# yaoyx689/RigGS

Measured on AMD Instinct MI355X. Metric: train iters/sec (deform+raster fwd+bwd), 300k Gaussians @800x800, higher is better.
Workload: dtype f32; 1 GPU; 300k Gaussians / 24-joint skeleton / 800x800, LBS-only, SH degree 3, anisotropic, one frame per GPU per step; num_gaussians=300000, num_joints=24, tile_instances_R=1963607, tile_lists=canonical: upstream's ceil(3 sigma) squares (the library default), parallelism=frames x1, launch=hipGraph replay

## Files before the change

riggs_amd/csrc/binning.hip:

```cpp
#include <stdlib.h>
#include <type_traits>
#include "raster_internal.h"
#include "color_job.h"

namespace riggs {


__device__ __forceinline__ int rect_tile(const ushort4 rc, int l, int grid_x) {
  const int w = rc.z - rc.x;
  const int ry = (int)(((float)l + 0.5f) * __builtin_amdgcn_rcpf((float)w));
  const int rx = l - ry * w;
  return (rc.y + ry) * grid_x + rc.x + rx;
}

__device__ __forceinline__ ushort4 unpack_rect(const uint2 w) {
  return make_ushort4((unsigned short)(w.x & 0xFFFFu), (unsigned short)(w.x >> 16), (unsigned short)(w.y & 0xFFFFu), (unsigned short)(w.y >> 16));
}
__device__ __forceinline__ ushort4 load_rect(const ushort4* p) { return unpack_rect(*reinterpret_cast<const uint2*>(p)); }

__global__ __launch_bounds__(1024) void bin_count_kernel(int N, int T, int grid_x, int g_per_block,
                                                        const uint32_t* __restrict__ order,
                                                        const ushort4* __restrict__ rect,
                                                        ushort4* __restrict__ srect ,
                                                        uint32_t* __restrict__ table) {
  extern __shared__ uint32_t s_hist[];
  for (int t = threadIdx.x; t < T; t += blockDim.x) s_hist[t] = 0u;
  __syncthreads();
  const int first = blockIdx.x * g_per_block;
  const int end = min(N, first + g_per_block);
  for (int s = first + threadIdx.x; s < end; s += blockDim.x) {
    const uint32_t g = order[s];
    const ushort4 rc = load_rect(rect + g);
    srect[s] = rc;
    if (rc.z == rc.x) continue;
    for (int y = rc.y; y < rc.w; y++)
      for (int x = rc.x; x < rc.z; x++) atomicAdd(&s_hist[y * grid_x + x], 1u);
  }
  __syncthreads();
  uint32_t* row = table + (size_t)blockIdx.x * T;
  for (int t = threadIdx.x; t < T; t += blockDim.x) row[t] = s_hist[t];
}

#define SCAN_SEG 16
#define SCAN_KEEP 32
__device__ __forceinline__ void bin_scan_body(int T, int n_chunks, uint32_t* __restrict__ table,
                                              uint32_t* __restrict__ tile_count) {
  __shared__ uint32_t s_seg[SCAN_SEG][64];
  const int tl = threadIdx.x & 63, seg = threadIdx.x >> 6;
  const int t = blockIdx.x * 64 + tl;
  const int per = (n_chunks + SCAN_SEG - 1) / SCAN_SEG;
  const int b0 = seg * per, b1 = min(n_chunks, b0 + per);
  uint32_t sum = 0;
  if (per <= SCAN_KEEP) {
    uint32_t v[SCAN_KEEP];
#pragma unroll
    for (int i = 0; i < SCAN_KEEP; i++) v[i] = (t < T && b0 + i < b1) ? table[(size_t)(b0 + i) * T + t] : 0u;
#pragma unroll
    for (int i = 0; i < SCAN_KEEP; i++) sum += v[i];
    s_seg[seg][tl] = sum;
    __syncthreads();
    uint32_t run = 0;
    for (int s2 = 0; s2 < seg; s2++) run += s_seg[s2][tl];
    if (t < T) {
#pragma unroll
      for (int i = 0; i < SCAN_KEEP; i++) {
        if (b0 + i < b1) table[(size_t)(b0 + i) * T + t] = run;
        run += v[i];
      }
      if (seg == SCAN_SEG - 1) tile_count[t] = run;
    }
    return;
  }
  if (t < T) for (int b = b0; b < b1; b++) sum += table[(size_t)b * T + t];
  s_seg[seg][tl] = sum;
  __syncthreads();
  uint32_t run = 0;
  for (int s2 = 0; s2 < seg; s2++) run += s_seg[s2][tl];
  if (t < T) {
    for (int b = b0; b < b1; b++) { const uint32_t c = table[(size_t)b * T + t]; table[(size_t)b * T + t] = run; run += c; }
    if (seg == SCAN_SEG - 1) tile_count[t] = run;
  }
}
__global__ __launch_bounds__(1024) void bin_scan_kernel(int T, int n_chunks, uint32_t* __restrict__ table,
                                                        uint32_t* __restrict__ tile_count) {
  bin_scan_body(T, n_chunks, table, tile_count);
}

__device__ void bin_offsets_body(int T, int64_t cap, const uint32_t* __restrict__ tile_count, const BinOut o,
                                 const uint32_t* __restrict__ total_src = nullptr, int n_total_src = 0) {
  uint2* __restrict__ ranges = o.ranges;
  uint32_t* __restrict__ slot_base = o.slot_base;
  uint32_t* __restrict__ tile_max = o.tile_max;
  uint32_t* __restrict__ counters = o.counters;
  uint32_t* __restrict__ fwd_items = o.fwd_items;
  uint32_t* __restrict__ fwd_empty = o.fwd_empty;
  uint32_t* __restrict__ fwd_ctr = o.fwd_ctr;
  __shared__ uint32_t s_wave[16], s_wwave[16];
  __shared__ uint32_t s_carry, s_wcarry;
  __shared__ uint32_t s_hist[33], s_cur[33], s_nempty;
  const int nthr = (int)blockDim.x;
  const int tid = threadIdx.x, lane = tid & 63, wave = tid >> 6;
  __shared__ int s_slot;
  if (tid == 0) { s_carry = 0u; s_nempty = 0u; s_wcarry = 0u; s_slot = RIGGS_HIST_SLOTS; }
  if (tid < 33) s_hist[tid] = 0u;
  const uint32_t slot_words = riggs_hist_slot_words((uint32_t)T);
  uint32_t* const hist_hdr = o.walk_hist;
  __syncthreads();
  if (o.viewmatrix) {
    for (int sl = tid; sl < RIGGS_HIST_SLOTS; sl += nthr) {
      const uint32_t* hs = hist_hdr + RIGGS_HIST_HDR + (size_t)sl * slot_words;
      bool ok = hs[T] == o.hist_stamp;
      for (int e = 0; e < 16 && ok; e++) ok = fabsf(o.viewmatrix[e] - __uint_as_float(hs[T + 2 + e])) <= o.view_tol;
      if (ok) atomicMin(&s_slot, sl);
    }
  } else if (tid == 0 && hist_hdr[RIGGS_HIST_HDR + T] == o.hist_stamp) s_slot = 0;
  __syncthreads();
  const bool slot_found = s_slot < RIGGS_HIST_SLOTS;
  const uint32_t cursor = hist_hdr[0];
  const int slot = slot_found ? s_slot : (o.viewmatrix ? (int)(cursor % RIGGS_HIST_SLOTS) : 0);
  uint32_t* __restrict__ walk_hist = hist_hdr + RIGGS_HIST_HDR + (size_t)slot * slot_words;
  const bool have_hist = o.wide_tiles > 0u && slot_found;
  __syncthreads();
  if (tid == 0) {
    hist_hdr[1] = (uint32_t)slot;
    if (!slot_found && o.viewmatrix) hist_hdr[0] = cursor + 1u;
  }
  uint32_t my_len[8];
#pragma unroll
  for (int k = 0; k < 8; k++) my_len[k] = 0u;
  for (int base = 0, pass = 0; base < T; base += nthr, pass++) {
    const int t = base + tid;
    const uint32_t c = (t < T) ? tile_count[t] : 0u;
    uint32_t v = c;
    for (int o2 = 1; o2 < 64; o2 <<= 1) {
      const uint32_t u = (uint32_t)__shfl_up((int)v, o2);
      if (lane >= o2) v += u;
    }
    const uint32_t prev = (have_hist && t < T) ? walk_hist[t] : 0u;
// ... 30 lines not shown
    __shared__ uint32_t s_tot;
    if (tid == 0) s_tot = 0u;
    __syncthreads();
    uint32_t part = 0;
    for (int k = tid; k < n_total_src; k += nthr) part += total_src[k];
    for (int o2 = 32; o2 > 0; o2 >>= 1) part += (uint32_t)__shfl_xor((int)part, o2);
    if (lane == 0) atomicAdd(&s_tot, part);
    __syncthreads();
    if (tid == 0) s_carry = s_tot;
    __syncthreads();
  }
  if (tid == 0) {
    const uint32_t R = s_carry;
    ranges[T] = make_uint2(0u, 0u);
    tile_max[T] = 0u;
    slot_base[T] = ((uint32_t)min((int64_t)R, cap) >> 6) + (uint32_t)T;
    counters[0] = R;
    counters[1] = (counters[1] & 2u) | (((int64_t)R > cap) ? 1u : 0u);
  }
  __syncthreads();
  if (tid < 32) {
    const uint32_t n_wide = s_hist[32];
    const uint32_t h = s_hist[31 - tid];
    uint32_t v = h;
    for (int o2 = 1; o2 < 32; o2 <<= 1) {
      const uint32_t u = (uint32_t)__shfl_up((int)v, o2);
      if (tid >= o2) v += u;
    }
    s_cur[31 - tid] = n_wide + v - h;
    if (tid == 0) s_cur[32] = 0u;
    if (tid == 31) { fwd_ctr[0] = n_wide + v; fwd_ctr[1] = n_wide; fwd_ctr[2] = s_nempty; fwd_ctr[64] = 0u; }
  }
  __syncthreads();
  auto emit = [&](uint32_t t, uint32_t len) { fwd_items[atomicAdd(&s_cur[(walk_hist[t] >> 31) ? 32 : 31 - __builtin_clz(len)], 1u)] = t; };
#pragma unroll
  for (int k = 0; k < 8; k++) {
    const int t = k * nthr + tid;
    if (t < T && my_len[k] > 0u) emit((uint32_t)t, my_len[k]);
  }
  for (int t = 8 * nthr + tid; t < T; t += nthr) {
    const uint2 r = ranges[t];
    if (r.y > r.x) emit((uint32_t)t, r.y - r.x);
  }
}

__global__ __launch_bounds__(1024) void bin_scatter_kernel(int N, int T, int grid_x, int64_t cap, int g_per_block, int g_per_wave,
                                                          const uint32_t* __restrict__ order,
                                                          const ushort4* __restrict__ srect ,
                                                          const uint32_t* __restrict__ table,
                                                          const uint32_t* __restrict__ tile_count,
                                                          uint32_t* __restrict__ point_list,
                                                          uint32_t* __restrict__ tile_keys, const BinOut out,
                                                          const int n_main, const ColorJob* __restrict__ job_rec, const int job_gpb) {
  extern __shared__ uint32_t s_mem[];
  if ((int)blockIdx.x == n_main) {
    bin_offsets_body(T, cap, tile_count, out);
    return;
  }
  if ((int)blockIdx.x > n_main) {
    const ColorJob job = *job_rec;
    color_block(job, (int)blockIdx.x - n_main - 1, job_gpb, reinterpret_cast<float*>(s_mem));
    return;
  }
  const int W = blockDim.x >> 6;
  uint32_t* s_base = s_mem;
  const int Tpad = (T + 1) & ~1;
  unsigned short* s_rel = reinterpret_cast<unsigned short*>(s_mem + T);
  uint32_t* s_rel32 = s_mem + T;
  const int tid = threadIdx.x, lane = tid & 63, wave = tid >> 6;
  const int first = blockIdx.x * g_per_block + wave * g_per_wave;
  const int end = min(N, min(first + g_per_wave, (blockIdx.x + 1) * g_per_block));
  auto load_batch = [&](int s0, uint32_t& g, uint32_t& n, ushort4& rc) {
    const int s = s0 + lane;
    g = 0u; n = 0u; rc = make_ushort4(0, 0, 0, 0);
    if (s < end) {
      g = order[s];
      rc = srect[s];
      n = (uint32_t)((int)(rc.z - rc.x) * (int)(rc.w - rc.y));
    }
  };
  uint32_t nx_g = 0u;
  uint2 nx_w = make_uint2(0u, 0u);
  if (first + lane < end) { nx_g = order[first + lane]; nx_w = *reinterpret_cast<const uint2*>(srect + first + lane); }
  const uint32_t* row = table + (size_t)blockIdx.x * T;
  uint32_t cq0[4], rq0[4];
#pragma unroll
  for (int k = 0; k < 4; k++) {
    const int t = k * (int)blockDim.x + tid;
    cq0[k] = (t < T) ? tile_count[t] : 0u;
    rq0[k] = (t < T) ? row[t] : 0u;
  }
  for (int e = tid; e < W * (Tpad >> 1); e += blockDim.x) s_rel32[e] = 0u;
  __syncthreads();
  ushort4 nx_rc = unpack_rect(nx_w);
  uint32_t nx_n = (uint32_t)((int)(nx_rc.z - nx_rc.x) * (int)(nx_rc.w - nx_rc.y));
  for (int s0 = first; s0 < end; s0 += 64) {
    uint32_t g = nx_g, n = nx_n;
    ushort4 rc = nx_rc;
    if (s0 != first) load_batch(s0, g, n, rc);
    if (n) {
      uint32_t* hist = s_rel32 + (size_t)wave * (Tpad >> 1);
      for (int y = rc.y; y < rc.w; y++)
        for (int x = rc.x; x < rc.z; x++) {
          const int t = y * grid_x + x;
          atomicAdd(&hist[t >> 1], 1u << (16 * (t & 1)));
        }
    }
  }
  __syncthreads();
  {
    __shared__ uint32_t s_wsum[16];
    __shared__ uint32_t s_run;
    if (tid == 0) s_run = 0u;
    __syncthreads();
    for (int base0 = 0; base0 < T; base0 += 4 * blockDim.x) {
      uint32_t cq[4], rq[4];
#pragma unroll
      for (int k = 0; k < 4; k++) {
        const int t = base0 + k * (int)blockDim.x + tid;
        if (base0 == 0) { cq[k] = cq0[k]; rq[k] = rq0[k]; continue; }
        cq[k] = (t < T) ? tile_count[t] : 0u;
        rq[k] = (t < T) ? row[t] : 0u;
      }
#pragma unroll
      for (int k = 0; k < 4; k++) {
        const int base = base0 + k * (int)blockDim.x;
        if (base >= T) break;
        const int t = base + tid;
        const uint32_t c = cq[k];
        uint32_t v = c;
        for (int o = 1; o < 64; o <<= 1) {
          const uint32_t u = (uint32_t)__shfl_up((int)v, o);
          if (lane >= o) v += u;
        }
        if (lane == 63) s_wsum[wave] = v;
        __syncthreads();
        uint32_t off = s_run;
        for (int w = 0; w < wave; w++) off += s_wsum[w];
        if (t < T) s_base[t] = off + v - c + rq[k];
        __syncthreads();
        if (tid == (int)blockDim.x - 1) s_run = off + v;
        __syncthreads();
      }
    }
  }
  for (int t = tid; t < T; t += blockDim.x) {
    uint32_t run = 0;
    for (int w = 0; w < W; w++) {
      const unsigned short c = s_rel[(size_t)w * Tpad + t];
      s_rel[(size_t)w * Tpad + t] = (unsigned short)run;
      run += c;
    }
  }
  __syncthreads();
  unsigned short* cur = s_rel + (size_t)wave * Tpad;
  const int slot4 = lane >> 4, l16 = lane & 15;
  for (int s0 = first; s0 < end; s0 += 64) {
    const uint32_t cur_g = nx_g, cur_n = nx_n;
    const ushort4 cur_rc = nx_rc;
    if (s0 + 64 < end) load_batch(s0 + 64, nx_g, nx_n, nx_rc);
    const uint64_t live = __builtin_amdgcn_ballot_w64(cur_n != 0u);
    const uint64_t large = __builtin_amdgcn_ballot_w64(cur_n > 16u);
    const uint64_t huge = __builtin_amdgcn_ballot_w64(cur_n > 32u);
    const int pk_xy = (int)cur_rc.x | ((int)cur_rc.y << 16), pk_zw = (int)cur_rc.z | ((int)cur_rc.w << 16);
#pragma unroll
    for (int q = 0; q < 16; q++) {
      if (((live >> (4 * q)) & 0xFull) == 0ull) continue;
      if (((large >> (4 * q)) & 0xFull) != 0ull && ((huge >> (4 * q)) & 0xFull) == 0ull) {
        const int slot2 = lane >> 5, l32 = lane & 31;
#pragma unroll
        for (int h = 0; h < 2; h++) {
          const int sa = 4 * q + 2 * h, sb = sa + 1;
          const int a0 = __builtin_amdgcn_readlane(pk_xy, sa), b0 = __builtin_amdgcn_readlane(pk_zw, sa);
          const int a1 = __builtin_amdgcn_readlane(pk_xy, sb), b1 = __builtin_amdgcn_readlane(pk_zw, sb);
          const int axy = slot2 ? a1 : a0, bzw = slot2 ? b1 : b0;
          const uint32_t g = (uint32_t)__shfl((int)cur_g, sa + slot2);
          const int rx0 = axy & 0xFFFF, ry0 = (int)((uint32_t)axy >> 16), rx1 = bzw & 0xFFFF, ry1 = (int)((uint32_t)bzw >> 16);
          const int w = rx1 - rx0;
          const int ry = (int)(((float)l32 + 0.5f) * __builtin_amdgcn_rcpf((float)w));
          const int x = rx0 + (l32 - ry * w), y = ry0 + ry;
          const bool valid = l32 < w * (ry1 - ry0);
          const bool in0 = x >= (a0 & 0xFFFF) && y >= (int)((uint32_t)a0 >> 16) && x < (b0 & 0xFFFF) && y < (int)((uint32_t)b0 >> 16);
          const bool in1 = x >= (a1 & 0xFFFF) && y >= (int)((uint32_t)a1 >> 16) && x < (b1 & 0xFFFF) && y < (int)((uint32_t)b1 >> 16);
          const int before = (slot2 && in0) ? 1 : 0;
          const bool last = slot2 || !in1;
          if (valid) {
            const int t = y * grid_x + x;
            const unsigned short rel = cur[t];
            if (last) cur[t] = (unsigned short)(rel + before + 1);
            const int64_t pos = (int64_t)s_base[t] + rel + before;
            if (pos < cap) { point_list[pos] = g; if (tile_keys) tile_keys[pos] = (uint32_t)t; }
          }
        }
        continue;
      }
      if (((large >> (4 * q)) & 0xFull) != 0ull) {
#pragma unroll
        for (int j = 0; j < 4; j++) {
          const int src = 4 * q + j;
          const int n = __builtin_amdgcn_readlane((int)cur_n, src);
          if (n == 0) continue;
          const uint32_t g = (uint32_t)__builtin_amdgcn_readlane((int)cur_g, src);
          const int r0 = __builtin_amdgcn_readlane(pk_xy, src), r1 = __builtin_amdgcn_readlane(pk_zw, src);
          ushort4 rc;
          rc.x = (unsigned short)(r0 & 0xFFFF); rc.y = (unsigned short)((uint32_t)r0 >> 16);
          rc.z = (unsigned short)(r1 & 0xFFFF); rc.w = (unsigned short)((uint32_t)r1 >> 16);
// ... 384 lines not shown
  {
    uint32_t pw[4];
#pragma unroll
    for (int w = 0; w < 4; w++) pw[w] = s_wbase[wave][w] + inc_scan[w] - cnt[w];
    place_lo = (uint64_t)pw[0] | ((uint64_t)pw[1] << 32);
    place_hi = (uint64_t)pw[2] | ((uint64_t)pw[3] << 32);
  }
#pragma unroll
  for (int i = 0; i < EPT; i++) {
    const uint32_t c = ev[i] >> 29;
    const bool hi = c >= 4u;
    const uint32_t sh = (c & 3u) * 16u;
    const uint32_t at = (uint32_t)((hi ? place_hi : place_lo) >> sh) & 0xFFFFu;
    const bool on = k_first + i < p.len;
    const uint64_t inc = on ? (1ull << sh) : 0ull;
    place_lo += hi ? 0ull : inc;
    place_hi += hi ? inc : 0ull;
    if (on) s_stage[at] = ev[i];
    __builtin_amdgcn_sched_barrier(0);
  }
  __syncthreads();
  uint32_t lstart[9];
#pragma unroll
  for (int q = 0; q < 9; q++) lstart[q] = s_lstart[q];
#pragma unroll 4
  for (uint32_t k = (uint32_t)tid; k < p.len; k += GTS_THREADS) {
    int c = 0;
#pragma unroll
    for (int q = 1; q < 8; q++) c += (k >= lstart[q]) ? 1 : 0;
    uint32_t ls = 0u;
#pragma unroll
    for (int q = 1; q < 8; q++) ls = (c == q) ? lstart[q] : ls;
    const int64_t pos = (int64_t)s_cur[c] + (k - ls);
    if (pos < cap) {
      point_list[pos] = s_stage[k] & 0x1FFFFFFFu;
      if (tile_keys) tile_keys[pos] = (uint32_t)(gy * grid_x + gx0 + c);
    }
  }
}

struct BinPlan { int g_per_block, g_per_wave, threads, n_chunks; size_t lds_scatter; };

static BinPlan bin_plan(int N, int T) {
  const int Tpad = (T + 1) & ~1;
  int W = 12;
  while (W > 1 && (size_t)T * 4 + (size_t)W * Tpad * 2 > 150 * 1024) W = (W + 1) >> 1;
  BinPlan p;
  p.threads = W * 64;
  int batches = (int)(((int64_t)N + (int64_t)W * 64 * 640 - 1) / ((int64_t)W * 64 * 640));
  batches = batches < 1 ? 1 : (batches > 16 ? 16 : batches);
  p.g_per_wave = 64 * batches;
  p.g_per_block = W * p.g_per_wave;
  p.n_chunks = (N + p.g_per_block - 1) / p.g_per_block;
  p.lds_scatter = (size_t)T * 4 + (size_t)W * Tpad * 2;
  return p;
}

static bool bin_grouped(int N, int T) {
  if (T > BIN_GROUPED_MIN_T) return true;
  const int forced = option(OPT_BIN_GROUPED);
  if (forced >= 0) return forced != 0 && T >= 64;
  return T >= BIN_GROUPED_AUTO_T && N >= BIN_GROUPED_AUTO_N;
}
bool binning_hosts_color(int N, int T, int sh_coeffs) {
  return option(OPT_COLOR_SIDE_JOBS) != 0 && N > 0 && sh_coeffs >= 1 && sh_coeffs <= 16 && T <= 65535 && !bin_grouped(N, T);
}
static void color_job_plan(const ColorJob* job_rec, int N, int T, int sh_coeffs, int threads, int& n_col, int& gpb, size_t& lds) {
  n_col = 0; gpb = 0;
  if (!job_rec || !binning_hosts_color(N, T, sh_coeffs)) return;
  const size_t row = (size_t)((sh_coeffs * 3) | 1) * 4;
  gpb = threads < 384 ? threads : 384;
  while (gpb > 64 && gpb * row > (lds > 256 * row ? lds : 256 * row)) gpb -= 64;
  if (gpb * row > lds) lds = gpb * row;
  n_col = (N + gpb - 1) / gpb;
}
struct GBinPlan { int G, gxg, W, g_per_block, g_per_wave, n_chunks; size_t lds; };
static GBinPlan gbin_plan(int N, int T, int grid_x) {
  GBinPlan p;
  p.gxg = (grid_x + 7) >> 3;
  const int grid_y = grid_x > 0 ? (T + grid_x - 1) / grid_x : 0;
  p.G = p.gxg * grid_y;
  int W = 16;
  while (W > 1 && (size_t)p.G * 4 + (size_t)W * p.G * 4 > 150 * 1024) W >>= 1;
  p.W = W;
  int batches = (int)(((int64_t)N + (int64_t)W * 64 * 512 - 1) / ((int64_t)W * 64 * 512));
  const int max_batches = 65535 / (W * 64 * 8);
  batches = batches < 1 ? 1 : (batches > max_batches ? max_batches : batches);
  p.g_per_wave = 64 * batches;
  p.g_per_block = W * p.g_per_wave;
  p.n_chunks = (N + p.g_per_block - 1) / p.g_per_block;
  p.lds = (size_t)p.G * 4 + (size_t)W * p.G * 4;
  return p;
}

size_t bin_table_bytes(int N, int T, int grid_x) {
  size_t grouped = 0, direct = 0;
  if (T >= 64) {
    GBinPlan p = gbin_plan(N > 0 ? N : 1, T, grid_x);
    grouped = align_up(((size_t)p.n_chunks + 1) * p.G * 4) + align_up((size_t)(p.G + 1) * 4) + align_up((size_t)(T + 1) * 4) +
              align_up((size_t)p.n_chunks * p.W * ((p.G + 1) & ~1) * 2) + align_up((size_t)(N > 0 ? N : 1) * 8);
  }
  if (T <= BIN_GROUPED_MIN_T) {
    BinPlan p = bin_plan(N > 0 ? N : 1, T);
    direct = align_up(((size_t)p.n_chunks + 1) * T * 4) + align_up((size_t)(T + 1) * 4) + align_up((size_t)(N > 0 ? N : 1) * 8);
  }
  return grouped > direct ? grouped : direct;
}
size_t bin_scratch_bytes(int64_t cap, int T, int grid_x) {
  GBinPlan p = gbin_plan(1, T, grid_x);
  const size_t c = (size_t)(cap > 0 ? cap : 1);
  return align_up(c * 4) + align_up((c / BIN_PART + (size_t)p.G + 2) * 8 * 4) + align_up((c / BIN_PART + (size_t)p.G + 2) * 16);
}

int launch_binning(int N, int T, int grid_x, int64_t cap, const uint32_t* order, const uint32_t* tiles,
                   const ushort4* rect, void* table_mem, void* scratch, uint32_t* point_list, uint32_t* tile_keys, const BinOut& out,
                   hipStream_t s, const ColorJob* job_rec, int job_sh_coeffs) {
  (void)tiles;
  if (T > 65535) { set_error("image too large: %d tiles (at most 65 535)", T); return 2; }
  char* mem = (char*)table_mem;
  static unsigned long long attr_done = 0ull;
  if (once_per_device(attr_done)) {
    (void)hipFuncSetAttribute(reinterpret_cast<const void*>(bin_scatter_kernel), hipFuncAttributeMaxDynamicSharedMemorySize, 158 * 1024);
    (void)hipFuncSetAttribute(reinterpret_cast<const void*>(bin_count_kernel), hipFuncAttributeMaxDynamicSharedMemorySize, 160 * 1024);
    (void)hipFuncSetAttribute(reinterpret_cast<const void*>(gbin_scatter_kernel), hipFuncAttributeMaxDynamicSharedMemorySize, 158 * 1024);
    (void)hipFuncSetAttribute(reinterpret_cast<const void*>(gbin_count_kernel), hipFuncAttributeMaxDynamicSharedMemorySize, 158 * 1024);
  }
  if (bin_grouped(N, T)) {
    const GBinPlan p = gbin_plan(N, T, grid_x);
    if (p.lds > 150 * 1024) { set_error("image too large: %d tile groups", p.G); return 2; }
    uint32_t* table = (uint32_t*)mem;
    uint32_t* group_count = (uint32_t*)(mem + align_up(((size_t)p.n_chunks + 1) * p.G * 4));
    uint32_t* tile_count = (uint32_t*)((char*)group_count + align_up((size_t)(p.G + 1) * 4));
    uint32_t* wave_start = (uint32_t*)((char*)tile_count + align_up((size_t)(T + 1) * 4));
    ushort4* srect = (ushort4*)((char*)wave_start + align_up((size_t)p.n_chunks * p.W * ((p.G + 1) & ~1) * 2));
    uint32_t* inter = (uint32_t*)scratch;
    uint32_t* part_hist = (uint32_t*)((char*)scratch + align_up((size_t)(cap > 0 ? cap : 1) * 4));
    const unsigned n_parts = (unsigned)((cap > 0 ? cap : 1) / BIN_PART + p.G + 1);
    uint4* part_tab = (uint4*)((char*)part_hist + align_up(((size_t)(cap > 0 ? cap : 1) / BIN_PART + (size_t)p.G + 2) * 8 * 4));
    hipLaunchKernelGGL(gbin_count_kernel, dim3(p.n_chunks), dim3(p.W * 64), (size_t)p.W * ((p.G + 1) & ~1) * 2, s, N, T, p.G, p.gxg,
                       p.g_per_block, p.g_per_wave, order, rect, srect, table, wave_start, tile_count);
    hipLaunchKernelGGL(bin_scan_kernel, dim3((p.G + 63) / 64), dim3(1024), 0, s, p.G, p.n_chunks, table, group_count);
    hipLaunchKernelGGL(gbin_scatter_kernel, dim3(p.n_chunks + 1), dim3(p.W * 64), p.lds, s, N, p.G, p.gxg, cap, p.g_per_block, p.g_per_wave,
                       order, srect, table, wave_start, group_count, inter, part_tab, n_parts);
    hipLaunchKernelGGL(gbin_tcount_kernel, dim3(n_parts), dim3(512), 0, s, p.gxg, grid_x, part_tab, inter, part_hist, tile_count);
    hipLaunchKernelGGL(gbin_tscatter_kernel, dim3(n_parts + 1), dim3(GTS_THREADS), 0, s, T, p.G, p.gxg, grid_x, cap, group_count, part_tab,
                       inter, part_hist, tile_count, point_list, tile_keys, out);
    return 0;
  }
  BinPlan p = bin_plan(N, T);
  uint32_t* table = (uint32_t*)mem;
  uint32_t* tile_count = (uint32_t*)(mem + align_up(((size_t)p.n_chunks + 1) * T * 4));
  ushort4* srect = (ushort4*)((char*)tile_count + align_up((size_t)(T + 1) * 4));
  if (p.lds_scatter > 150 * 1024) {
    set_error("image too large: %d tiles", T);
    return 2;
  }
  hipLaunchKernelGGL(bin_count_kernel, dim3(p.n_chunks), dim3(p.threads), (size_t)T * 4, s, N, T, grid_x, p.g_per_block,
                     order, rect, srect, table);
  hipLaunchKernelGGL(bin_scan_kernel, dim3((T + 63) / 64), dim3(1024), 0, s, T, p.n_chunks, table, tile_count);
  int n_col = 0, gpb = 0;
  size_t lds = p.lds_scatter;
  color_job_plan(job_rec, N, T, job_sh_coeffs, p.threads, n_col, gpb, lds);
  hipLaunchKernelGGL(bin_scatter_kernel, dim3(p.n_chunks + 1 + n_col), dim3(p.threads), lds, s, N, T, grid_x, cap,
                     p.g_per_block, p.g_per_wave, order, srect, table, tile_count, point_list, tile_keys, out, p.n_chunks, job_rec, gpb);
  return 0;
}


#define RS_BITS 12
#define RS_BINS (1 << RS_BITS)
#define RS_CHUNK 2048
#define RS_CHUNK_BIG 8192
#ifndef RS_BIG_MIN_N
#define RS_BIG_MIN_N 1000000
#endif
#define RS_SC_WAVES 8

struct RsBufs {
  const uint32_t* k_in;
  uint2 *a, *b;
  uint32_t* v_out;
};
__device__ __forceinline__ void rs_route(const RsBufs& r, int pass, bool three, const uint2*& src, uint2*& dst) {
  if (pass == 0) { src = nullptr; dst = three ? r.b : r.a; }
  else if (pass == 1) { src = three ? r.b : r.a; dst = three ? r.a : nullptr; }
  else { src = r.a; dst = nullptr; }
}

template <int CHUNK>
__global__ __launch_bounds__(CHUNK / 8) void rs_count_kernel(int N, int pass, RsBufs bufs, uint32_t* __restrict__ table,
                                                             const uint32_t* __restrict__ part, int n_part,
                                                             uint32_t* __restrict__ counters, uint32_t* __restrict__ arrivals) {
  constexpr int NT = CHUNK / 8, NW = NT / 64;
  __shared__ uint32_t s_hist[RS_BINS];
  __shared__ uint32_t s_w[NW], s_lo[NW], s_hi[NW];
  const int first = blockIdx.x * CHUNK;
  uint32_t k0[CHUNK / NT];
#pragma unroll
  for (int k = 0; k < CHUNK / NT; k++) {
    const int i = first + k * NT + threadIdx.x;
    k0[k] = (pass == 0 && i < N) ? bufs.k_in[i] : 0u;
  }
  bool three;
  if (pass == 0) {
    uint32_t v = 0, lo = 0xFFu, hi = 0u;
    for (int i = threadIdx.x; i < n_part; i += NT) {
      v += part[i];
      const uint32_t tb = part[n_part + i];
      lo = min(lo, tb >> 8); hi = max(hi, tb & 0xFFu);
    }
    for (int o = 32; o > 0; o >>= 1) {
      v += (uint32_t)__shfl_xor((int)v, o);
      lo = min(lo, (uint32_t)__shfl_xor((int)lo, o)); hi = max(hi, (uint32_t)__shfl_xor((int)hi, o));
    }
    if ((threadIdx.x & 63) == 0) { s_w[threadIdx.x >> 6] = v; s_lo[threadIdx.x >> 6] = lo; s_hi[threadIdx.x >> 6] = hi; }
    __syncthreads();
    uint32_t total = 0;
    lo = 0xFFu; hi = 0u;
#pragma unroll
    for (int w = 0; w < NW; w++) { total += s_w[w]; lo = min(lo, s_lo[w]); hi = max(hi, s_hi[w]); }
    three = hi > lo;
    if (blockIdx.x == gridDim.x - 1 && threadIdx.x == 0) {
      counters[0] = total; counters[1] = 0u; counters[2] = three ? 1u : 0u; counters[3] = 0u;
      arrivals[0] = 0u;
    }
  } else {
    three = counters[2] != 0u;
  }
  const uint2* src; uint2* dst;
  rs_route(bufs, pass, three, src, dst);
  const int shift = pass * RS_BITS;
  if (src) {
#pragma unroll
    for (int k = 0; k < CHUNK / NT; k++) k0[k] = src[min(first + k * NT + (int)threadIdx.x, N - 1)].x;
  }
  for (int b = threadIdx.x; b < RS_BINS; b += NT) s_hist[b] = 0u;
  __syncthreads();
#pragma unroll
  for (int k = 0; k < CHUNK / NT; k++) {
    const int i = first + k * NT + threadIdx.x;
    if (i < N) atomicAdd(&s_hist[(k0[k] >> shift) & (RS_BINS - 1)], 1u);
  }
  __syncthreads();
  uint32_t* row = table + (size_t)blockIdx.x * RS_BINS;
  for (int b = threadIdx.x; b < RS_BINS; b += NT) row[b] = s_hist[b];
}

__global__ __launch_bounds__(1024) void rs_scan_kernel(int n_chunks, uint32_t* __restrict__ table, uint32_t* __restrict__ bin_count,
                                                       const uint32_t* __restrict__ counters, int pass) {
  (void)counters; (void)pass;
  bin_scan_body(RS_BINS, n_chunks, table, bin_count);
}

#define RS3_BINS 256
#define RS3_MAX_WG 512
typedef __attribute__((address_space(1))) uint32_t rs_gu32;
template <int CHUNK>
__device__ void rs_third_pass_body(int N, int n_chunks, const RsBufs& bufs, uint32_t* __restrict__ table3,
                                   uint32_t* __restrict__ counters, const int G ) {
  __shared__ uint32_t s_hist[RS3_BINS];
  __shared__ uint32_t s_start[RS3_BINS];
  __shared__ unsigned short s_wave[RS_SC_WAVES][RS3_BINS];
  __shared__ int s_fail;
  const uint2* src = bufs.a;
  uint32_t* vd = bufs.v_out;
  constexpr int NT = RS_SC_WAVES * 64, STEPS = CHUNK / NT;
  const int tid = threadIdx.x, lane = tid & 63, wave = tid >> 6;
  for (int chunk = blockIdx.x; chunk < n_chunks; chunk += G) {
    if (tid < RS3_BINS) s_hist[tid] = 0u;
    __syncthreads();
#pragma unroll
    for (int st = 0; st < STEPS; st++) {
      const int i = chunk * CHUNK + wave * (64 * STEPS) + st * 64 + lane;
      if (i < N) atomicAdd(&s_hist[src[i].x >> 24], 1u);
    }
    __syncthreads();
    if (tid < RS3_BINS)
      __hip_atomic_store((rs_gu32*)(table3 + (size_t)chunk * RS3_BINS + tid), s_hist[tid], __ATOMIC_RELAXED, __HIP_MEMORY_SCOPE_AGENT);
    __syncthreads();
  }
  asm volatile("s_waitcnt vmcnt(0)" ::: "memory");
  if (tid == 0) s_fail = 0;
  __syncthreads();
  if (tid == 0) {
    __hip_atomic_fetch_add((rs_gu32*)(counters + 3), 1u, __ATOMIC_RELAXED, __HIP_MEMORY_SCOPE_AGENT);
    uint32_t spins = 0;
    while (__hip_atomic_load((rs_gu32*)(counters + 3), __ATOMIC_RELAXED, __HIP_MEMORY_SCOPE_AGENT) < (uint32_t)G) {
      __builtin_amdgcn_s_sleep(8);
      if (++spins > (1u << 22)) { s_fail = 1; break; }
    }
  }
  __syncthreads();
  if (s_fail) {
    if (tid == 0) atomicOr(counters + 1, 2u);
    return;
  }
  for (int chunk = blockIdx.x; chunk < n_chunks; chunk += G) {
    for (int e = tid; e < RS_SC_WAVES * RS3_BINS / 2; e += NT) reinterpret_cast<uint32_t*>(&s_wave[0][0])[e] = 0u;
    if (tid < RS3_BINS) {
      uint32_t total = 0, before = 0;
      for (int c = 0; c < n_chunks; c += 4) {
        uint32_t v[4];
#pragma unroll
        for (int u = 0; u < 4; u++)
          v[u] = (c + u < n_chunks) ? __hip_atomic_load((rs_gu32*)(table3 + (size_t)(c + u) * RS3_BINS + tid), __ATOMIC_RELAXED, __HIP_MEMORY_SCOPE_AGENT) : 0u;
#pragma unroll
        for (int u = 0; u < 4; u++) { total += v[u]; if (c + u < chunk) before += v[u]; }
      }
      s_hist[tid] = total;
      s_start[tid] = before;
    }
    __syncthreads();
    uint32_t key[STEPS], val[STEPS];
    int dig[STEPS];
#pragma unroll
    for (int st = 0; st < STEPS; st++) {
      const int i = chunk * CHUNK + wave * (64 * STEPS) + st * 64 + lane;
      key[st] = 0u; val[st] = 0u; dig[st] = -1;
      if (i < N) {
        const uint2 kv = src[i];
        key[st] = kv.x; val[st] = kv.y;
        dig[st] = (int)(key[st] >> 24);
        atomicAdd(reinterpret_cast<uint32_t*>(&s_wave[wave][0]) + (dig[st] >> 1), 1u << (16 * (dig[st] & 1)));
      }
    }
    if (wave == 0) {
      uint32_t c4[4], t = 0;
#pragma unroll
      for (int u = 0; u < 4; u++) { c4[u] = s_hist[lane * 4 + u]; t += c4[u]; }
      uint32_t v = t;
      for (int o = 1; o < 64; o <<= 1) {
        const uint32_t u2 = (uint32_t)__shfl_up((int)v, o);
        if (lane >= o) v += u2;
      }
      uint32_t run = v - t;
#pragma unroll
      for (int u = 0; u < 4; u++) { s_start[lane * 4 + u] += run; run += c4[u]; }
    }
    __syncthreads();
    for (int b = tid; b < RS3_BINS; b += NT) {
      unsigned short r = 0;
#pragma unroll
      for (int w = 0; w < RS_SC_WAVES; w++) { const unsigned short cw = s_wave[w][b]; s_wave[w][b] = r; r += cw; }
    }
    __syncthreads();
    unsigned short* cur = s_wave[wave];
#pragma unroll
    for (int st = 0; st < STEPS; st++) {
      const bool on = dig[st] >= 0;
      uint64_t same = __builtin_amdgcn_ballot_w64(on);
#pragma unroll
      for (int b = 0; b < 8; b++) {
        const uint64_t vote = __builtin_amdgcn_ballot_w64(on && ((dig[st] >> b) & 1));
        same &= ((dig[st] >> b) & 1) ? vote : ~vote;
      }
      if (on) {
        const uint64_t below = same & ((1ull << lane) - 1ull);
        const uint32_t rank = (uint32_t)__builtin_popcountll(below);
        const unsigned short base = cur[dig[st]];
        const uint32_t pos = s_start[dig[st]] + base + rank;
        vd[pos] = val[st];
        if ((same >> lane) >> 1 == 0ull) cur[dig[st]] = base + (unsigned short)__builtin_popcountll(same);
      }
    }
    __syncthreads();
  }
}

template <int CHUNK>
__global__ __launch_bounds__(RS_SC_WAVES * 64) void rs_scatter_kernel(int N, int pass, RsBufs bufs,
                                                                      const uint32_t* __restrict__ table ,
                                                                      const uint32_t* __restrict__ bin_count,
                                                                      uint32_t* __restrict__ counters,
                                                                      uint32_t* __restrict__ table3 ,
                                                                      uint32_t* __restrict__ arrivals, int g3) {
  __shared__ uint32_t s_start[RS_BINS];
  __shared__ unsigned short s_wave[RS_SC_WAVES][RS_BINS];
  __shared__ uint32_t s_part[RS_SC_WAVES];
  const bool three = counters[2] != 0u;
  const uint2* src; uint2* dst;
  rs_route(bufs, pass, three, src, dst);
  const int shift = pass * RS_BITS;
  const int tid = threadIdx.x, lane = tid & 63, wave = tid >> 6;
  constexpr int NT = RS_SC_WAVES * 64, PER = RS_BINS / NT;
  constexpr int STEPS = CHUNK / NT;
  const int wfirst = blockIdx.x * CHUNK + wave * (64 * STEPS);
  const uint32_t* row = table + (size_t)blockIdx.x * RS_BINS;
  uint32_t rw[PER];
#pragma unroll
  for (int k = 0; k < PER; k++) rw[k] = row[tid * PER + k];
  uint32_t c[PER], tsum = 0;
#pragma unroll
  for (int k = 0; k < PER; k++) c[k] = bin_count[tid * PER + k];
  uint32_t key[STEPS], val[STEPS];
  if (src) {
#pragma unroll
    for (int st = 0; st < STEPS; st++) {
      const uint2 kv = src[min(wfirst + st * 64 + lane, N - 1)];
      key[st] = kv.x; val[st] = kv.y;
    }
  } else {
#pragma unroll
    for (int st = 0; st < STEPS; st++) {
      const int i = wfirst + st * 64 + lane;
      key[st] = bufs.k_in[min(i, N - 1)]; val[st] = (uint32_t)i;
    }
  }
#pragma unroll
  for (int k = 0; k < PER; k++) tsum += c[k];
  uint32_t v = tsum;
  for (int o = 1; o < 64; o <<= 1) {
    const uint32_t u = (uint32_t)__shfl_up((int)v, o);
    if (lane >= o) v += u;
  }
  if (lane == 63) s_part[wave] = v;
  for (int e = tid; e < RS_SC_WAVES * RS_BINS / 2; e += NT) reinterpret_cast<uint32_t*>(&s_wave[0][0])[e] = 0u;
  __syncthreads();
  uint32_t run = v - tsum;
  for (int w = 0; w < wave; w++) run += s_part[w];
#pragma unroll
  for (int k = 0; k < PER; k++) { s_start[tid * PER + k] = run + rw[k]; run += c[k]; }
  int dig[STEPS];
#pragma unroll
  for (int st = 0; st < STEPS; st++) {
    const int i = wfirst + st * 64 + lane;
    dig[st] = -1;
    if (i < N) {
      dig[st] = (int)((key[st] >> shift) & (RS_BINS - 1));
      atomicAdd(reinterpret_cast<uint32_t*>(&s_wave[wave][0]) + (dig[st] >> 1), 1u << (16 * (dig[st] & 1)));
    }
  }
  __syncthreads();
  for (int b = tid; b < RS_BINS; b += NT) {
    unsigned short r = 0;
#pragma unroll
    for (int w = 0; w < RS_SC_WAVES; w++) { const unsigned short cw = s_wave[w][b]; s_wave[w][b] = r; r += cw; }
  }
  __syncthreads();
  unsigned short* cur = s_wave[wave];
#pragma unroll
  for (int st = 0; st < STEPS; st++) {
    const bool on = dig[st] >= 0;
    uint64_t same = __builtin_amdgcn_ballot_w64(on);
#pragma unroll
    for (int b = 0; b < RS_BITS; b++) {
      const uint64_t vote = __builtin_amdgcn_ballot_w64(on && ((dig[st] >> b) & 1));
      same &= ((dig[st] >> b) & 1) ? vote : ~vote;
    }
    if (on) {
      const uint64_t below = same & ((1ull << lane) - 1ull);
      const uint32_t rank = (uint32_t)__builtin_popcountll(below);
      const unsigned short base = cur[dig[st]];
      const uint32_t pos = s_start[dig[st]] + base + rank;
      if (dst) dst[pos] = make_uint2(key[st], val[st]); else bufs.v_out[pos] = val[st];
      if ((same >> lane) >> 1 == 0ull) cur[dig[st]] = base + (unsigned short)__builtin_popcountll(same);
    }
  }
  if (pass != 1 || !three) return;
  __shared__ int s_late;
  __atomic_thread_fence(__ATOMIC_RELEASE);
  __syncthreads();
  if (tid == 0) {
    s_late = 0;
    __hip_atomic_fetch_add((rs_gu32*)arrivals, 1u, __ATOMIC_RELEASE, __HIP_MEMORY_SCOPE_AGENT);
    if ((int)blockIdx.x < g3) {
      uint32_t spins = 0;
      while (__hip_atomic_load((rs_gu32*)arrivals, __ATOMIC_RELAXED, __HIP_MEMORY_SCOPE_AGENT) < gridDim.x) {
        __builtin_amdgcn_s_sleep(8);
        if (++spins > (1u << 22)) { s_late = 1; break; }
      }
    }
  }
  __syncthreads();
  if ((int)blockIdx.x >= g3) return;
  if (s_late) {
    if (tid == 0) atomicOr(counters + 1, 2u);
    return;
  }
  __atomic_thread_fence(__ATOMIC_ACQUIRE);
  rs_third_pass_body<CHUNK>(N, (int)gridDim.x, bufs, table3, counters, g3);
}

size_t depth_sort_table_bytes(int N) {
  const size_t n = (size_t)(N > 0 ? N : 1), chunks = (n + RS_CHUNK - 1) / RS_CHUNK;
  return align_up((chunks + 1) * RS_BINS * 4) + align_up(RS_BINS * 4) + 2 * align_up(n * 8) + 256;
}

template <int CHUNK>
static int launch_depth_sort_t(int N, const uint32_t* keys_in, uint32_t* keys_out, uint32_t* vals_out, void* table_mem,
                               const uint32_t* block_info, uint32_t* counters, hipStream_t s) {
  const int chunks = (N + CHUNK - 1) / CHUNK;
  char* mem = (char*)table_mem;
  uint32_t* table = (uint32_t*)mem;
  uint32_t* bin_count = (uint32_t*)(mem + align_up(((size_t)((N + RS_CHUNK - 1) / RS_CHUNK) + 1) * RS_BINS * 4));
  RsBufs b;
  (void)keys_out;
  b.k_in = keys_in;
  b.a = (uint2*)((char*)bin_count + align_up(RS_BINS * 4));
  b.b = (uint2*)((char*)b.a + align_up((size_t)(N > 0 ? N : 1) * 8));
  b.v_out = vals_out;
  static int rs3_grid = 0;
  if (rs3_grid == 0) {
    int per_cu = 0, dev = 0, cus = 0;
    if (hipOccupancyMaxActiveBlocksPerMultiprocessor(&per_cu, reinterpret_cast<const void*>(rs_scatter_kernel<CHUNK>), RS_SC_WAVES * 64, 0) != hipSuccess ||
        hipGetDevice(&dev) != hipSuccess || hipDeviceGetAttribute(&cus, hipDeviceAttributeMultiprocessorCount, dev) != hipSuccess) {
      per_cu = 1; cus = 64; (void)hipGetLastError();
    }
    const int resident = (per_cu > 0 ? per_cu : 1) * (cus > 0 ? cus : 1);
    rs3_grid = resident / 2 > 0 ? resident / 2 : 1;
    if (rs3_grid > RS3_MAX_WG) rs3_grid = RS3_MAX_WG;
  }
  uint32_t* arrivals = (uint32_t*)((char*)b.b + align_up((size_t)(N > 0 ? N : 1) * 8));
  for (int pass = 0; pass < 2; pass++) {
    hipLaunchKernelGGL(rs_count_kernel<CHUNK>, dim3(chunks), dim3(CHUNK / 8), 0, s, N, pass, b, table, block_info, (N + 255) / 256, counters,
                       arrivals);
    hipLaunchKernelGGL(rs_scan_kernel, dim3((RS_BINS + 63) / 64), dim3(1024), 0, s, chunks, table, bin_count, counters, pass);
    hipLaunchKernelGGL(rs_scatter_kernel<CHUNK>, dim3(chunks), dim3(RS_SC_WAVES * 64), 0, s, N, pass, b, table, bin_count, counters,
                       table, arrivals, chunks < rs3_grid ? chunks : rs3_grid);
  }
  return 0;
}

int launch_depth_sort(int N, const uint32_t* keys_in, uint32_t* keys_out, uint32_t* vals_out, void* table_mem,
                      const uint32_t* block_info, uint32_t* counters, hipStream_t s) {
  if (N >= RS_BIG_MIN_N) return launch_depth_sort_t<RS_CHUNK_BIG>(N, keys_in, keys_out, vals_out, table_mem, block_info, counters, s);
  return launch_depth_sort_t<RS_CHUNK>(N, keys_in, keys_out, vals_out, table_mem, block_info, counters, s);
}

}
```

Measured before the change: 3025 iters/s.

## Vectorize LDS per-wave offset scans and cut barriers in binning/sort scatter

Reworks the bin scatter kernel's block-wide prefix over tiles so it uses one barrier per group of 4 tile batches, a readlane-based cross-wave scan and a register carry, replacing three barriers per batch. Per-wave u16 count-to-offset scans in the bin scatter and radix-sort scatters become 8- or 4-wide packed 16-bit adds with 16-byte LDS accesses, and the LDS layout is realigned for this. The scan kernels' tile width per block becomes a template parameter, which changes the grid and register-kept chunk depth. This adds alignment assumptions and a slightly larger LDS budget check.

```diff
diff --git a/riggs_amd/csrc/binning.hip b/riggs_amd/csrc/binning.hip
--- a/riggs_amd/csrc/binning.hip
+++ b/riggs_amd/csrc/binning.hip
@@ -17,6 +17,35 @@
   return make_ushort4((unsigned short)(w.x & 0xFFFFu), (unsigned short)(w.x >> 16), (unsigned short)(w.y & 0xFFFFu), (unsigned short)(w.y >> 16));
 }
 __device__ __forceinline__ ushort4 load_rect(const ushort4* p) { return unpack_rect(*reinterpret_cast<const uint2*>(p)); }
+
+__device__ __forceinline__ uint32_t pk_add_u16(uint32_t a, uint32_t b) {
+  typedef unsigned short us2 __attribute__((ext_vector_type(2)));
+  return __builtin_bit_cast(uint32_t, __builtin_bit_cast(us2, a) + __builtin_bit_cast(us2, b));
+}
+
+__host__ __device__ __forceinline__ int bin_rel_stride(int T) { return (T + 7) & ~7; }
+template <int WC>
+__device__ __forceinline__ void rel_counts_to_offsets4(uint2* __restrict__ rel64, int row64 , int W, int tid, int nthr) {
+  for (int q = tid; q < row64; q += nthr) {
+    uint2 r = make_uint2(0u, 0u);
+    if constexpr (WC > 0) {
+      uint2 cw[WC];
+#pragma unroll
+      for (int w = 0; w < WC; w++) cw[w] = rel64[(size_t)w * row64 + q];
+#pragma unroll
+      for (int w = 0; w < WC; w++) {
+        rel64[(size_t)w * row64 + q] = r;
+        r.x = pk_add_u16(r.x, cw[w].x); r.y = pk_add_u16(r.y, cw[w].y);
+      }
+    } else {
+      for (int w = 0; w < W; w++) {
+        const uint2 c = rel64[(size_t)w * row64 + q];
+        rel64[(size_t)w * row64 + q] = r;
+        r.x = pk_add_u16(r.x, c.x); r.y = pk_add_u16(r.y, c.y);
+      }
+    }
+  }
+}
 
 __global__ __launch_bounds__(1024) void bin_count_kernel(int N, int T, int grid_x, int g_per_block,
                                                         const uint32_t* __restrict__ order,
@@ -41,33 +70,42 @@
   for (int t = threadIdx.x; t < T; t += blockDim.x) row[t] = s_hist[t];
 }
 
-#define SCAN_SEG 16
-#define SCAN_KEEP 32
+#define SCAN_THREADS 1024
+#define SCAN_CHUNKS 512
+#ifndef BIN_SCAN_TILES
+#define BIN_SCAN_TILES 64
+#endif
+#ifndef RS_SCAN_TILES
+#define RS_SCAN_TILES 32
+#endif
+template <int TILES>
 __device__ __forceinline__ void bin_scan_body(int T, int n_chunks, uint32_t* __restrict__ table,
                                               uint32_t* __restrict__ tile_count) {
-  __shared__ uint32_t s_seg[SCAN_SEG][64];
-  const int tl = threadIdx.x & 63, seg = threadIdx.x >> 6;
-  const int t = blockIdx.x * 64 + tl;
-  const int per = (n_chunks + SCAN_SEG - 1) / SCAN_SEG;
+  constexpr int SEGS = SCAN_THREADS / TILES, KEEP = SCAN_CHUNKS / SEGS;
+  static_assert(TILES * SEGS == SCAN_THREADS && KEEP * SEGS == SCAN_CHUNKS && (TILES & (TILES - 1)) == 0, "the split");
+  __shared__ uint32_t s_seg[SEGS][TILES];
+  const int tl = threadIdx.x & (TILES - 1), seg = threadIdx.x / TILES;
+  const int t = blockIdx.x * TILES + tl;
+  const int per = (n_chunks + SEGS - 1) / SEGS;
   const int b0 = seg * per, b1 = min(n_chunks, b0 + per);
   uint32_t sum = 0;
-  if (per <= SCAN_KEEP) {
-    uint32_t v[SCAN_KEEP];
-#pragma unroll
-    for (int i = 0; i < SCAN_KEEP; i++) v[i] = (t < T && b0 + i < b1) ? table[(size_t)(b0 + i) * T + t] : 0u;
-#pragma unroll
-    for (int i = 0; i < SCAN_KEEP; i++) sum += v[i];
+  if (per <= KEEP) {
+    uint32_t v[KEEP];
+#pragma unroll
+    for (int i = 0; i < KEEP; i++) v[i] = (t < T && b0 + i < b1) ? table[(size_t)(b0 + i) * T + t] : 0u;
+#pragma unroll
+    for (int i = 0; i < KEEP; i++) sum += v[i];
     s_seg[seg][tl] = sum;
     __syncthreads();
     uint32_t run = 0;
     for (int s2 = 0; s2 < seg; s2++) run += s_seg[s2][tl];
     if (t < T) {
 #pragma unroll
-      for (int i = 0; i < SCAN_KEEP; i++) {
+      for (int i = 0; i < KEEP; i++) {
         if (b0 + i < b1) table[(size_t)(b0 + i) * T + t] = run;
         run += v[i];
       }
-      if (seg == SCAN_SEG - 1) tile_count[t] = run;
+      if (seg == SEGS - 1) tile_count[t] = run;
     }
     return;
   }
@@ -78,12 +116,13 @@
   for (int s2 = 0; s2 < seg; s2++) run += s_seg[s2][tl];
   if (t < T) {
     for (int b = b0; b < b1; b++) { const uint32_t c = table[(size_t)b * T + t]; table[(size_t)b * T + t] = run; run += c; }
-    if (seg == SCAN_SEG - 1) tile_count[t] = run;
-  }
-}
-__global__ __launch_bounds__(1024) void bin_scan_kernel(int T, int n_chunks, uint32_t* __restrict__ table,
-                                                        uint32_t* __restrict__ tile_count) {
-  bin_scan_body(T, n_chunks, table, tile_count);
+    if (seg == SEGS - 1) tile_count[t] = run;
+  }
+}
+static inline unsigned bin_scan_grid(int T, int tiles) { return (unsigned)((T + tiles - 1) / tiles); }
+__global__ __launch_bounds__(SCAN_THREADS) void bin_scan_kernel(int T, int n_chunks, uint32_t* __restrict__ table,
+                                                                uint32_t* __restrict__ tile_count) {
+  bin_scan_body<BIN_SCAN_TILES>(T, n_chunks, table, tile_count);
 }
 
 __device__ void bin_offsets_body(int T, int64_t cap, const uint32_t* __restrict__ tile_count, const BinOut o,
@@ -220,7 +259,7 @@
                                                           uint32_t* __restrict__ point_list,
                                                           uint32_t* __restrict__ tile_keys, const BinOut out,
                                                           const int n_main, const ColorJob* __restrict__ job_rec, const int job_gpb) {
-  extern __shared__ uint32_t s_mem[];
+  extern __shared__ __attribute__((aligned(16))) uint32_t s_mem[];
   if ((int)blockIdx.x == n_main) {
     bin_offsets_body(T, cap, tile_count, out);
     return;
@@ -231,10 +270,10 @@
     return;
   }
   const int W = blockDim.x >> 6;
-  uint32_t* s_base = s_mem;
-  const int Tpad = (T + 1) & ~1;
-  unsigned short* s_rel = reinterpret_cast<unsigned short*>(s_mem + T);
-  uint32_t* s_rel32 = s_mem + T;
+  const int Tpad = bin_rel_stride(T);
+  unsigned short* s_rel = reinterpret_cast<unsigned short*>(s_mem);
+  uint32_t* s_rel32 = s_mem;
+  uint32_t* s_base = s_mem + W * (Tpad >> 1);
   const int tid = threadIdx.x, lane = tid & 63, wave = tid >> 6;
   const int first = blockIdx.x * g_per_block + wave * g_per_wave;
   const int end = min(N, min(first + g_per_wave, (blockIdx.x + 1) * g_per_block));
@@ -258,7 +297,7 @@
     cq0[k] = (t < T) ? tile_count[t] : 0u;
     rq0[k] = (t < T) ? row[t] : 0u;
   }
-  for (int e = tid; e < W * (Tpad >> 1); e += blockDim.x) s_rel32[e] = 0u;
+  for (int e = tid; e < W * (Tpad >> 3); e += blockDim.x) reinterpret_cast<uint4*>(s_rel32)[e] = make_uint4(0u, 0u, 0u, 0u);
   __syncthreads();
   ushort4 nx_rc = unpack_rect(nx_w);
   uint32_t nx_n = (uint32_t)((int)(nx_rc.z - nx_rc.x) * (int)(nx_rc.w - nx_rc.y));
@@ -275,14 +314,11 @@
         }
     }
   }
-  __syncthreads();
   {
-    __shared__ uint32_t s_wsum[16];
-    __shared__ uint32_t s_run;
-    if (tid == 0) s_run = 0u;
-    __syncthreads();
-    for (int base0 = 0; base0 < T; base0 += 4 * blockDim.x) {
-      uint32_t cq[4], rq[4];
+    __shared__ uint32_t s_wsum[2][64];
+    uint32_t carry = 0u;
+    for (int base0 = 0, grp = 0; base0 < T; base0 += 4 * blockDim.x, grp ^= 1) {
+      uint32_t cq[4], rq[4], v[4];
 #pragma unroll
       for (int k = 0; k < 4; k++) {
         const int t = base0 + k * (int)blockDim.x + tid;
@@ -292,34 +328,32 @@
       }
 #pragma unroll
       for (int k = 0; k < 4; k++) {
-        const int base = base0 + k * (int)blockDim.x;
-        if (base >= T) break;
-        const int t = base + tid;
-        const uint32_t c = cq[k];
-        uint32_t v = c;
+        v[k] = cq[k];
         for (int o = 1; o < 64; o <<= 1) {
-          const uint32_t u = (uint32_t)__shfl_up((int)v, o);
-          if (lane >= o) v += u;
+          const uint32_t u = (uint32_t)__shfl_up((int)v[k], o);
+          if (lane >= o) v[k] += u;
         }
-        if (lane == 63) s_wsum[wave] = v;
-        __syncthreads();
-        uint32_t off = s_run;
-        for (int w = 0; w < wave; w++) off += s_wsum[w];
-        if (t < T) s_base[t] = off + v - c + rq[k];
-        __syncthreads();
-        if (tid == (int)blockDim.x - 1) s_run = off + v;
-        __syncthreads();
-      }
-    }
-  }
-  for (int t = tid; t < T; t += blockDim.x) {
-    uint32_t run = 0;
-    for (int w = 0; w < W; w++) {
-      const unsigned short c = s_rel[(size_t)w * Tpad + t];
-      s_rel[(size_t)w * Tpad + t] = (unsigned short)run;
-      run += c;
-    }
-  }
+        if (lane == 63) s_wsum[grp][k * 16 + wave] = v[k];
+      }
+      __syncthreads();
+      const uint32_t tot = ((lane & 15) < W) ? s_wsum[grp][lane] : 0u;
+      uint32_t inc = tot;
+      for (int o = 1; o < 64; o <<= 1) {
+        const uint32_t u = (uint32_t)__shfl_up((int)inc, o);
+        if (lane >= o) inc += u;
+      }
+      const uint32_t exc = inc - tot;
+#pragma unroll
+      for (int k = 0; k < 4; k++) {
+        const int t = base0 + k * (int)blockDim.x + tid;
+        const uint32_t off = carry + (uint32_t)__builtin_amdgcn_readlane((int)exc, k * 16 + wave);
+        if (t < T) s_base[t] = off + v[k] - cq[k] + rq[k];
+      }
+      carry += (uint32_t)__builtin_amdgcn_readlane((int)inc, 63);
+    }
+  }
+  if (W == 12) rel_counts_to_offsets4<12>(reinterpret_cast<uint2*>(s_rel32), Tpad >> 2, W, tid, (int)blockDim.x);
+  else rel_counts_to_offsets4<0>(reinterpret_cast<uint2*>(s_rel32), Tpad >> 2, W, tid, (int)blockDim.x);
   __syncthreads();
   unsigned short* cur = s_rel + (size_t)wave * Tpad;
   const int slot4 = lane >> 4, l16 = lane & 15;
@@ -810,7 +844,7 @@
   p.g_per_wave = 64 * batches;
   p.g_per_block = W * p.g_per_wave;
   p.n_chunks = (N + p.g_per_block - 1) / p.g_per_block;
-  p.lds_scatter = (size_t)T * 4 + (size_t)W * Tpad * 2;
+  p.lds_scatter = (size_t)T * 4 + (size_t)W * bin_rel_stride(T) * 2;
   return p;
 }
 
@@ -897,7 +931,7 @@
     uint4* part_tab = (uint4*)((char*)part_hist + align_up(((size_t)(cap > 0 ? cap : 1) / BIN_PART + (size_t)p.G + 2) * 8 * 4));
     hipLaunchKernelGGL(gbin_count_kernel, dim3(p.n_chunks), dim3(p.W * 64), (size_t)p.W * ((p.G + 1) & ~1) * 2, s, N, T, p.G, p.gxg,
                        p.g_per_block, p.g_per_wave, order, rect, srect, table, wave_start, tile_count);
-    hipLaunchKernelGGL(bin_scan_kernel, dim3((p.G + 63) / 64), dim3(1024), 0, s, p.G, p.n_chunks, table, group_count);
+    hipLaunchKernelGGL(bin_scan_kernel, dim3(bin_scan_grid(p.G, BIN_SCAN_TILES)), dim3(SCAN_THREADS), 0, s, p.G, p.n_chunks, table, group_count);
     hipLaunchKernelGGL(gbin_scatter_kernel, dim3(p.n_chunks + 1), dim3(p.W * 64), p.lds, s, N, p.G, p.gxg, cap, p.g_per_block, p.g_per_wave,
                        order, srect, table, wave_start, group_count, inter, part_tab, n_parts);
     hipLaunchKernelGGL(gbin_tcount_kernel, dim3(n_parts), dim3(512), 0, s, p.gxg, grid_x, part_tab, inter, part_hist, tile_count);
@@ -909,13 +943,13 @@
   uint32_t* table = (uint32_t*)mem;
   uint32_t* tile_count = (uint32_t*)(mem + align_up(((size_t)p.n_chunks + 1) * T * 4));
   ushort4* srect = (ushort4*)((char*)tile_count + align_up((size_t)(T + 1) * 4));
-  if (p.lds_scatter > 150 * 1024) {
+  if (p.lds_scatter > 150 * 1024 + 192) {
     set_error("image too large: %d tiles", T);
     return 2;
   }
   hipLaunchKernelGGL(bin_count_kernel, dim3(p.n_chunks), dim3(p.threads), (size_t)T * 4, s, N, T, grid_x, p.g_per_block,
                      order, rect, srect, table);
-  hipLaunchKernelGGL(bin_scan_kernel, dim3((T + 63) / 64), dim3(1024), 0, s, T, p.n_chunks, table, tile_count);
+  hipLaunchKernelGGL(bin_scan_kernel, dim3(bin_scan_grid(T, BIN_SCAN_TILES)), dim3(SCAN_THREADS), 0, s, T, p.n_chunks, table, tile_count);
   int n_col = 0, gpb = 0;
   size_t lds = p.lds_scatter;
   color_job_plan(job_rec, N, T, job_sh_coeffs, p.threads, n_col, gpb, lds);
@@ -933,6 +967,24 @@
 #define RS_BIG_MIN_N 1000000
 #endif
 #define RS_SC_WAVES 8
+
+template <int ROWS, int BINS>
+__device__ __forceinline__ void wave_rows_zero8(unsigned short* tab, int b0) {
+#pragma unroll
+  for (int w = 0; w < ROWS; w++) *reinterpret_cast<uint4*>(tab + w * BINS + b0) = make_uint4(0u, 0u, 0u, 0u);
+}
+template <int ROWS, int BINS>
+__device__ __forceinline__ void wave_rows_counts_to_offsets8(unsigned short* tab, int b0) {
+  uint4 cw[ROWS];
+#pragma unroll
+  for (int w = 0; w < ROWS; w++) cw[w] = *reinterpret_cast<const uint4*>(tab + w * BINS + b0);
+  uint4 r = make_uint4(0u, 0u, 0u, 0u);
+#pragma unroll
+  for (int w = 0; w < ROWS; w++) {
+    *reinterpret_cast<uint4*>(tab + w * BINS + b0) = r;
+    r.x = pk_add_u16(r.x, cw[w].x); r.y = pk_add_u16(r.y, cw[w].y); r.z = pk_add_u16(r.z, cw[w].z); r.w = pk_add_u16(r.w, cw[w].w);
+  }
+}
 
 struct RsBufs {
   const uint32_t* k_in;
@@ -1004,10 +1056,10 @@
   for (int b = threadIdx.x; b < RS_BINS; b += NT) row[b] = s_hist[b];
 }
 
-__global__ __launch_bounds__(1024) void rs_scan_kernel(int n_chunks, uint32_t* __restrict__ table, uint32_t* __restrict__ bin_count,
+__global__ __launch_bounds__(SCAN_THREADS) void rs_scan_kernel(int n_chunks, uint32_t* __restrict__ table, uint32_t* __restrict__ bin_count,
                                                        const uint32_t* __restrict__ counters, int pass) {
   (void)counters; (void)pass;
-  bin_scan_body(RS_BINS, n_chunks, table, bin_count);
+  bin_scan_body<RS_SCAN_TILES>(RS_BINS, n_chunks, table, bin_count);
 }
 
 #define RS3_BINS 256
@@ -1018,7 +1070,7 @@
                                    uint32_t* __restrict__ counters, const int G ) {
   __shared__ uint32_t s_hist[RS3_BINS];
   __shared__ uint32_t s_start[RS3_BINS];
-  __shared__ unsigned short s_wave[RS_SC_WAVES][RS3_BINS];
+  __shared__ __attribute__((aligned(16))) unsigned short s_wave[RS_SC_WAVES][RS3_BINS];
   __shared__ int s_fail;
   const uint2* src = bufs.a;
   uint32_t* vd = bufs.v_out;
@@ -1054,7 +1106,7 @@
     return;
   }
   for (int chunk = blockIdx.x; chunk < n_chunks; chunk += G) {
-    for (int e = tid; e < RS_SC_WAVES * RS3_BINS / 2; e += NT) reinterpret_cast<uint32_t*>(&s_wave[0][0])[e] = 0u;
+    if (tid >= NT - RS3_BINS / 8) wave_rows_zero8<RS_SC_WAVES, RS3_BINS>(&s_wave[0][0], (tid - (NT - RS3_BINS / 8)) * 8);
     if (tid < RS3_BINS) {
       uint32_t total = 0, before = 0;
       for (int c = 0; c < n_chunks; c += 4) {
@@ -1096,11 +1148,7 @@
       for (int u = 0; u < 4; u++) { s_start[lane * 4 + u] += run; run += c4[u]; }
     }
     __syncthreads();
-    for (int b = tid; b < RS3_BINS; b += NT) {
-      unsigned short r = 0;
-#pragma unroll
-      for (int w = 0; w < RS_SC_WAVES; w++) { const unsigned short cw = s_wave[w][b]; s_wave[w][b] = r; r += cw; }
-    }
+    if (tid < RS3_BINS / 8) wave_rows_counts_to_offsets8<RS_SC_WAVES, RS3_BINS>(&s_wave[0][0], tid * 8);
     __syncthreads();
     unsigned short* cur = s_wave[wave];
 #pragma unroll
@@ -1132,8 +1180,8 @@
                                                                       uint32_t* __restrict__ counters,
                                                                       uint32_t* __restrict__ table3 ,
                                                                       uint32_t* __restrict__ arrivals, int g3) {
-  __shared__ uint32_t s_start[RS_BINS];
-  __shared__ unsigned short s_wave[RS_SC_WAVES][RS_BINS];
+  __shared__ __attribute__((aligned(16))) uint32_t s_start[RS_BINS];
+  __shared__ __attribute__((aligned(16))) unsigned short s_wave[RS_SC_WAVES][RS_BINS];
   __shared__ uint32_t s_part[RS_SC_WAVES];
   const bool three = counters[2] != 0u;
   const uint2* src; uint2* dst;
@@ -1141,6 +1189,8 @@
   const int shift = pass * RS_BITS;
   const int tid = threadIdx.x, lane = tid & 63, wave = tid >> 6;
   constexpr int NT = RS_SC_WAVES * 64, PER = RS_BINS / NT;
+  static_assert(PER == 8, "a thread's bins are one 16-byte access of a u16 row");
+  static_assert(CHUNK < 65536, "packed 16-bit counters: a chunk adds at most CHUNK to a bin, a wave 64 x STEPS");
   constexpr int STEPS = CHUNK / NT;
   const int wfirst = blockIdx.x * CHUNK + wave * (64 * STEPS);
   const uint32_t* row = table + (size_t)blockIdx.x * RS_BINS;
@@ -1172,7 +1222,7 @@
     if (lane >= o) v += u;
   }
   if (lane == 63) s_part[wave] = v;
-  for (int e = tid; e < RS_SC_WAVES * RS_BINS / 2; e += NT) reinterpret_cast<uint32_t*>(&s_wave[0][0])[e] = 0u;
+  wave_rows_zero8<RS_SC_WAVES, RS_BINS>(&s_wave[0][0], tid * PER);
   __syncthreads();
   uint32_t run = v - tsum;
   for (int w = 0; w < wave; w++) run += s_part[w];
@@ -1189,11 +1239,7 @@
     }
   }
   __syncthreads();
-  for (int b = tid; b < RS_BINS; b += NT) {
-    unsigned short r = 0;
-#pragma unroll
-    for (int w = 0; w < RS_SC_WAVES; w++) { const unsigned short cw = s_wave[w][b]; s_wave[w][b] = r; r += cw; }
-  }
+  wave_rows_counts_to_offsets8<RS_SC_WAVES, RS_BINS>(&s_wave[0][0], tid * PER);
   __syncthreads();
   unsigned short* cur = s_wave[wave];
 #pragma unroll
@@ -1272,7 +1318,7 @@
   for (int pass = 0; pass < 2; pass++) {
     hipLaunchKernelGGL(rs_count_kernel<CHUNK>, dim3(chunks), dim3(CHUNK / 8), 0, s, N, pass, b, table, block_info, (N + 255) / 256, counters,
                        arrivals);
-    hipLaunchKernelGGL(rs_scan_kernel, dim3((RS_BINS + 63) / 64), dim3(1024), 0, s, chunks, table, bin_count, counters, pass);
+    hipLaunchKernelGGL(rs_scan_kernel, dim3(bin_scan_grid(RS_BINS, RS_SCAN_TILES)), dim3(SCAN_THREADS), 0, s, chunks, table, bin_count, counters, pass);
     hipLaunchKernelGGL(rs_scatter_kernel<CHUNK>, dim3(chunks), dim3(RS_SC_WAVES * 64), 0, s, N, pass, b, table, bin_count, counters,
                        table, arrivals, chunks < rs3_grid ? chunks : rs3_grid);
   }
```

After: 3091 iters/s (median of 6 runs). 2.2% higher.
